# microsoft/protnote

Measured on AMD Instinct MI355X. Metric: protein-label pairs/sec (fwd+bwd), higher is better.
Workload: dtype f32

## Files before the change

### include/protnote_hip.h

```cpp
#ifndef PROTNOTE_HIP_H
#define PROTNOTE_HIP_H

#include <stddef.h>
#include <stdint.h>

#ifdef __cplusplus
extern "C" {
#endif

#define PN_MAX_BLOCKS 16
#define PN_MAX_LAYERS 8
#define PN_LABEL_F32 0
#define PN_LABEL_I64 1
#define PN_LABEL_U8 2

const char* pn_last_error(void);
int pn_version(void);
const char* pn_build_hash(void);

typedef struct pn_bn {
  const float* weight;
  const float* bias;
  float* running_mean;
  float* running_var;
// ... 179 lines not shown

#define PN_ADAM_WS_BYTES 32768
int pn_clip_adam_step(float* w, const float* g, float* m, float* v, long n, float max_norm, float lr, float beta1,
                      float beta2, float eps, float weight_decay, int step, float* norm_out, void* ws,
                      size_t ws_bytes, void* stream);

int pn_clip_sgd_step(float* w, const float* g, float* momentum_buf, long n, float max_norm, float lr, float momentum,
                     float weight_decay, int step, float* norm_out, void* ws, size_t ws_bytes, void* stream);

int pn_transpose(const float* src, long ld_src, int rows, int cols, float* dst, long ld_dst, void* stream);

int pn_gemm_tn(const float* A, long lda, const float* Bm, long ldb, float* C, long ldc, long R, int M, int N,
               void* ws, size_t ws_bytes, void* stream);

int pn_onehot_batch(const uint8_t* ids, const int64_t* offsets, int B, int A, int Lmax, float* onehots,
                    int64_t* lengths, void* stream);


int pn_ap_append(const float* scores, int ld_s, const void* labels, int label_kind, int ld_y, int B, int N_L,
                 uint32_t* keys, uint8_t* hits, long long cap, long long n0, void* stream);
size_t pn_ap_ws_bytes(int N_L, long long n, long long cap, int micro);
int pn_ap_compute(const uint32_t* keys, const uint8_t* hits, int N_L, long long n, long long cap, double* ap,
                  long long* npos, double* micro_ap, long long* micro_npos, void* ws, size_t ws_bytes, void* stream);

size_t pn_ap_partial_ws_bytes(long long m);
int pn_ap_partial(const uint32_t* keys, const uint8_t* hits, long long m, long long tp_before, long long k_before,
                  double* partial, long long* npos, void* ws, size_t ws_bytes, void* stream);

int pn_binned_hist_update(const float* scores, int ld_s, const void* labels, int label_kind, int ld_y, int B, int N_L,
                          const float* thresholds, int T, unsigned long long* pos_hist, unsigned long long* all_hist,
                          void* stream);
int pn_binned_auprc(unsigned long long* pos_hist, unsigned long long* all_hist, int N_L, int T, double* out,
                    long long* npos, int with_micro, void* stream);

int pn_set_math_mode(int mode);

int pn_set_mlp_materialize(int on);

typedef int (*pn_sync_hook)(long n_doubles, void* user);
int pn_set_sync_bn(pn_sync_hook hook, void* user, double* stage, long stage_doubles, int world);
int pn_get_math_mode(void);

int pn_set_backward_math(int mode);
int pn_get_backward_math(void);

int pn_set_forward_math(int mode);
int pn_get_forward_math(void);
int pn_set_fwd_staged(int on);
int pn_set_bf16_mfma16(int on);
int pn_set_bwd_deep(int mask);

int pn_set_f32_dma(int on);
int pn_set_b3_dma(int on);

int pn_set_encoder_f64(int on);

int pn_set_conv1_gather(int on);

int pn_dropout_mask(unsigned seed, int stream, float p, long rows, int cols, float* out, void* stream_);

int pn_prof_begin(void);
int pn_prof_end(int max_kinds, int* kinds, long* counts, double* total_ms, double* total_flops);

size_t pn_gemm_nt_stats_ws_bytes(int M, int N);
int pn_gemm_nt(const float* A, long lda, const float* W, long ldw, float* C, long ldc, int M, int N, int K,
               const float* bias, const float* a_scale, const float* a_shift, double* col_sum,
               double* col_sumsq, int tile_variant, void* ws, size_t ws_bytes, void* stream);

#ifdef __cplusplus
}
#endif
#endif
```

### protnote_amd/_lib.py

```python
import ctypes as C
import os

import torch

_HERE = os.path.dirname(os.path.abspath(__file__))
LIB_PATH = os.path.join(_HERE, "libprotnote_hip.so")

PN_MAX_BLOCKS = 16
PN_MAX_LAYERS = 8
PN_ADAM_WS_BYTES = 32768
fp = C.POINTER(C.c_float)


class pn_bn(C.Structure):
    _fields_ = [("weight", C.c_void_p), ("bias", C.c_void_p), ("running_mean", C.c_void_p),
                ("running_var", C.c_void_p)]


class pn_res_block(C.Structure):
    _fields_ = [("bn1", pn_bn), ("conv_a_w", C.c_void_p), ("conv_a_b", C.c_void_p), ("bn2", pn_bn),
                ("conv_b_w", C.c_void_p), ("conv_b_b", C.c_void_p)]


class pn_encoder(C.Structure):
# ... 108 lines not shown
    "pn_loss_fwd_bwd": (C.c_int, [C.c_void_p, C.c_void_p, C.c_void_p, C.c_int, C.c_int, C.c_int, C.c_float,
                                  C.c_float, C.c_float, C.c_float, C.c_float, C.c_void_p, C.c_void_p, C.c_void_p,
                                  C.c_void_p, C.c_void_p, C.c_int, C.c_void_p, C.c_float, C.c_void_p, C.c_size_t,
                                  C.c_void_p]),
    "pn_loss_fwd_bwd_t": (C.c_int, [C.c_void_p, C.c_void_p, C.c_int, C.c_int, C.c_int, C.c_int, C.c_float,
                                    C.c_float, C.c_float, C.c_float, C.c_float, C.c_void_p, C.c_void_p, C.c_void_p,
                                    C.c_void_p, C.c_void_p, C.c_int, C.c_void_p, C.c_float, C.c_void_p, C.c_size_t,
                                    C.c_void_p]),
    "pn_tp_fn_fp_t": (C.c_int, [C.c_void_p, C.c_void_p, C.c_int, C.c_int, C.c_int, C.c_float, C.c_void_p,
                                C.c_void_p, C.c_void_p, C.c_void_p]),
    "pn_supcon_ws_bytes": (C.c_size_t, [C.c_int]),
    "pn_supcon_fwd_bwd": (C.c_int, [C.c_void_p, C.c_void_p, C.c_void_p, C.c_int, C.c_int, C.c_void_p, C.c_void_p,
                                    C.c_void_p, C.c_size_t, C.c_void_p]),
    "pn_tp_fn_fp": (C.c_int, [C.c_void_p, C.c_void_p, C.c_void_p, C.c_int, C.c_int, C.c_float, C.c_void_p,
                              C.c_void_p, C.c_void_p, C.c_void_p]),
    "pn_clip_adam_step": (C.c_int, [C.c_void_p, C.c_void_p, C.c_void_p, C.c_void_p, C.c_long, C.c_float, C.c_float,
                                    C.c_float, C.c_float, C.c_float, C.c_float, C.c_int, C.c_void_p, C.c_void_p,
                                    C.c_size_t, C.c_void_p]),
    "pn_clip_sgd_step": (C.c_int, [C.c_void_p, C.c_void_p, C.c_void_p, C.c_long, C.c_float, C.c_float, C.c_float,
                                   C.c_float, C.c_int, C.c_void_p, C.c_void_p, C.c_size_t, C.c_void_p]),
    "pn_transpose": (C.c_int, [C.c_void_p, C.c_long, C.c_int, C.c_int, C.c_void_p, C.c_long, C.c_void_p]),
    "pn_gemm_tn": (C.c_int, [C.c_void_p, C.c_long, C.c_void_p, C.c_long, C.c_void_p, C.c_long, C.c_long, C.c_int,
                             C.c_int, C.c_void_p, C.c_size_t, C.c_void_p]),
    "pn_onehot_batch": (C.c_int, [C.c_void_p, C.c_void_p, C.c_int, C.c_int, C.c_int, C.c_void_p, C.c_void_p,
                                  C.c_void_p]),
    "pn_ap_append": (C.c_int, [C.c_void_p, C.c_int, C.c_void_p, C.c_int, C.c_int, C.c_int, C.c_int, C.c_void_p,
                               C.c_void_p, C.c_longlong, C.c_longlong, C.c_void_p]),
    "pn_ap_ws_bytes": (C.c_size_t, [C.c_int, C.c_longlong, C.c_longlong, C.c_int]),
    "pn_ap_compute": (C.c_int, [C.c_void_p, C.c_void_p, C.c_int, C.c_longlong, C.c_longlong, C.c_void_p, C.c_void_p,
                                C.c_void_p, C.c_void_p, C.c_void_p, C.c_size_t, C.c_void_p]),
    "pn_ap_partial_ws_bytes": (C.c_size_t, [C.c_longlong]),
    "pn_ap_partial": (C.c_int, [C.c_void_p, C.c_void_p, C.c_longlong, C.c_longlong, C.c_longlong, C.c_void_p, C.c_void_p,
                                C.c_void_p, C.c_size_t, C.c_void_p]),
    "pn_binned_hist_update": (C.c_int, [C.c_void_p, C.c_int, C.c_void_p, C.c_int, C.c_int, C.c_int, C.c_int,
                                        C.c_void_p, C.c_int, C.c_void_p, C.c_void_p, C.c_void_p]),
    "pn_binned_auprc": (C.c_int, [C.c_void_p, C.c_void_p, C.c_int, C.c_int, C.c_void_p, C.c_void_p, C.c_int,
                                  C.c_void_p]),
    "pn_dropout_mask": (C.c_int, [C.c_uint, C.c_int, C.c_float, C.c_long, C.c_int, C.c_void_p, C.c_void_p]),
    "pn_set_math_mode": (C.c_int, [C.c_int]),
    "pn_set_mlp_materialize": (C.c_int, [C.c_int]),
    "pn_set_sync_bn": (C.c_int, [C.c_void_p, C.c_void_p, C.c_void_p, C.c_long, C.c_int]),
    "pn_get_math_mode": (C.c_int, []),
    "pn_set_backward_math": (C.c_int, [C.c_int]),
    "pn_get_backward_math": (C.c_int, []),
    "pn_set_forward_math": (C.c_int, [C.c_int]),
    "pn_get_forward_math": (C.c_int, []),
    "pn_set_fwd_staged": (C.c_int, [C.c_int]),
    "pn_set_bf16_mfma16": (C.c_int, [C.c_int]),
    "pn_set_bwd_deep": (C.c_int, [C.c_int]),
    "pn_set_f32_dma": (C.c_int, [C.c_int]),
    "pn_set_encoder_f64": (C.c_int, [C.c_int]),
    "pn_set_conv1_gather": (C.c_int, [C.c_int]),
    "pn_set_b3_dma": (C.c_int, [C.c_int]),
    "pn_prof_begin": (C.c_int, []),
    "pn_prof_end": (C.c_int, [C.c_int, C.POINTER(C.c_int), C.POINTER(C.c_long), C.POINTER(C.c_double),
                              C.POINTER(C.c_double)]),
    "pn_gemm_nt": (C.c_int, [C.c_void_p, C.c_long, C.c_void_p, C.c_long, C.c_void_p, C.c_long, C.c_int, C.c_int,
                             C.c_int, C.c_void_p, C.c_void_p, C.c_void_p, C.c_void_p, C.c_void_p, C.c_int,
                             C.c_void_p, C.c_size_t, C.c_void_p]),
    "pn_gemm_nt_stats_ws_bytes": (C.c_size_t, [C.c_int, C.c_int]),
    "pn_loss_ws_bytes": (C.c_size_t, [C.c_int, C.c_int]),
}


def exported_symbols():
    return sorted(_SIGS)


def _ensure_current():
    from . import build

    have_src = os.path.isdir(build.CSRC) and os.path.exists(os.path.join(build.CSRC, "protnote_hip.hip"))
    if os.path.exists(LIB_PATH) and (not have_src or os.environ.get("PN_SKIP_HASH_CHECK") == "1"):
        return
    if os.path.exists(LIB_PATH) and not build.stale():
        return
    why = "is missing" if not os.path.exists(LIB_PATH) else (
        f"was built from other sources (binary {build.embedded_hash()}, csrc/ {build.csrc_hash()})")
    if not build.have_hipcc():
        raise RuntimeError(f"{LIB_PATH} {why} and hipcc is not available to rebuild it; build it with "
                           "`python -m protnote_amd.build` (protnote_amd has no CPU/eager fallback)")
    try:
        build.build_lib(verbose=False)
    except Exception as exc:
        raise RuntimeError(f"{LIB_PATH} {why} and could not be rebuilt ({exc}); build it with "
                           "`python -m protnote_amd.build` (protnote_amd has no CPU/eager fallback)") from exc


def build_hash() -> str:
    return lib().pn_build_hash().decode()


def lib():
    global _lib
    if _lib is None:
        _ensure_current()
        l = C.CDLL(LIB_PATH)
        for name, (res, args) in _SIGS.items():
            fn = getattr(l, name)
            fn.restype = res
            fn.argtypes = args
        _lib = l
        mode = os.environ.get("PN_MATH_MODE")
        if mode:
            set_math_mode(mode)
        mode = os.environ.get("PN_BACKWARD_MATH")
# ... 135 lines not shown
```

### protnote_amd/csrc/abi_heads_eval.hpp

```cpp
extern "C" size_t pn_mlp_rows_ws_bytes(const pn_mlp* m, int rows) {
  size_t b = 0;
  int hmax = 0;
  for (int i = 0; i + 1 < m->nlayers; ++i) hmax = m->dims[i + 1] > hmax ? m->dims[i + 1] : hmax;
  b += 2 * al256((size_t)rows * hmax * sizeof(float));
  b += 2 * al256((size_t)hmax * sizeof(float));
  return b;
}

extern "C" int pn_mlp_rows_fwd_eval(const pn_mlp* m, const float* x, int ldx, int rows, float* y, void* ws,
                                    size_t ws_bytes, void* stream) {
  PN_OK(math_field_check(m->math_mode, "pn_mlp_rows_fwd_eval"));
  MathScope math_scope(m->math_mode);
  hipStream_t st = (hipStream_t)stream;
  if (m->nlayers < 1 || m->nlayers > PN_MAX_LAYERS) return fail("mlp: bad layer count %d", m->nlayers);
  for (int i = 0; i <= m->nlayers; ++i)
    if (i < m->nlayers && m->dims[i] % 4 != 0) return fail("mlp: dims[%d]=%d not a multiple of 4", i, m->dims[i]);
  if (ldx % 4 != 0) return fail("mlp: ldx %% 4 != 0");
  int hmax = 0;
  for (int i = 0; i + 1 < m->nlayers; ++i) hmax = m->dims[i + 1] > hmax ? m->dims[i + 1] : hmax;
  Bump bp(ws, ws_bytes);
  float* buf[2];
  buf[0] = bp.take<float>((size_t)rows * hmax);
  buf[1] = bp.take<float>((size_t)rows * hmax);
  float* s = bp.take<float>(hmax);
// ... 452 lines not shown
    p.task_ns = ns;
    grid = dim3(tn_task_grid(ns), 1);
    if (SYNC && sync_ws != nullptr && ns * 4 * 4 <= TN_SYNC_INTS) {
      HIP_OK(hipMemsetAsync(sync_ws, 0, (size_t)ns * 4 * 4 * sizeof(int), st));
      p.task_sync = sync_ws;
    }
  }
  {
    ProfScope ps(100 + TA_PLAIN * 10 + TB, 2.0 * (double)R_all * (double)p.M * (double)p.N, st);
    hipLaunchKernelGGL(kern, grid, dim3(512), TN_FAST_LDS_BYTES, st, p);
    if (tail != 0) {
      auto tk = gemm_tn_kernel<TA_PLAIN, TB, false>;
      static bool tattr[64] = {false};
      if (dev < 64 && !tattr[dev]) {
        HIP_OK(hipFuncSetAttribute((const void*)tk, hipFuncAttributeMaxDynamicSharedMemorySize, TN_LDS_BYTES));
        tattr[dev] = true;
      }
      TnParams t = p;
      t.R = R_all; t.row_base = R_all - tail; t.rows_per_split = 32;
      t.Cpart = part + (size_t)ns * p.M * p.N; t.ldc = p.N; t.task_ns = 0; t.task_sync = nullptr;
      hipLaunchKernelGGL(tk, dim3((unsigned)((p.M / 128) * (p.N / 128)), 1), dim3(256), TN_LDS_BYTES, st, t);
    }
  }
  HIP_OK(hipGetLastError());
  if (ns > 1 || tail != 0) {
    hipLaunchKernelGGL(k_splitk_reduce, dim3(nblk((long)p.M * p.N, 256)), dim3(256), 0, st, (const float*)part,
                       ns + (tail != 0 ? 1 : 0), p.M, p.N, (long)p.N, dst, ldd);
    HIP_OK(hipGetLastError());
  }
  return 0;
}

template <int TB, int NP = 3, bool TR = false, bool ABF16 = false>
static int launch_tn_bf16x3(TnParams p, float* dst, long ldd, float* part, size_t part_cap_floats, hipStream_t st) {
  void (*kern)(TnParams) = nullptr;
  constexpr bool SYNC = TR && TB == TB_AFFINE_RELU;
  void (*kern_alt)(TnParams) = nullptr;
  if constexpr (TR) {
    kern = gemm_tn_bf16tr_kernel<TB, ABF16, SYNC, true>;
    kern_alt = gemm_tn_bf16tr_kernel<TB, ABF16, SYNC, false>;
  } else {
    kern = gemm_tn_bf16x3_kernel<TB, NP>;
  }
  constexpr int LDS = TR ? TN_BF16TR_LDS_BYTES : 2 * 512 * 36 * (int)sizeof(float);
  static std::atomic<bool> attr_done[64];
  int dev = 0;
  HIP_OK(hipGetDevice(&dev));
  if (dev < 64 && !attr_done[dev]) {
    HIP_OK(hipFuncSetAttribute((const void*)kern, hipFuncAttributeMaxDynamicSharedMemorySize, LDS));
    if (kern_alt != nullptr) HIP_OK(hipFuncSetAttribute((const void*)kern_alt, hipFuncAttributeMaxDynamicSharedMemorySize, LDS));
    attr_done[dev] = true;
  }
  if (kern_alt != nullptr && !g_bf16_m16.load()) kern = kern_alt;
  int ns = tn_pick_split(p.R, p.M, p.N, part_cap_floats, 256, 1);
  if (ns == 1) {
    p.Cpart = dst;
    p.ldc = ldd;
    p.rows_per_split = (p.R + 31) / 32 * 32;
  } else {
    if (part == nullptr) return fail("gemm_tn: no partial buffer");
    p.Cpart = part;
    p.ldc = p.N;
    long rps = (p.R + ns - 1) / ns;
    p.rows_per_split = (rps + 31) / 32 * 32;
    ns = (int)((p.R + p.rows_per_split - 1) / p.rows_per_split);
  }
  const unsigned tiles = (unsigned)((p.M / 256) * (p.N / 256));
  dim3 grid(tiles, (unsigned)ns);
  p.task_ns = 0;
  int* sync_ws = p.task_sync;
  p.task_sync = nullptr;
  if (p.M == 3072 && p.N == 3072 && ns >= 2) {
    p.task_ns = ns;
    grid = dim3(tn_task_grid(ns), 1);
    if (SYNC && sync_ws != nullptr && ns * 4 * 4 <= TN_SYNC_INTS) {
      HIP_OK(hipMemsetAsync(sync_ws, 0, (size_t)ns * 4 * 4 * sizeof(int), st));
      p.task_sync = sync_ws;
    }
  }
  {
    ProfScope ps((NP == 3 ? 1100 : 1600) + TB, 2.0 * (double)p.R * (double)p.M * (double)p.N, st);
    hipLaunchKernelGGL(kern, grid, dim3(512), LDS, st, p);
  }
  HIP_OK(hipGetLastError());
  if (ns > 1) {
    hipLaunchKernelGGL(k_splitk_reduce, dim3(nblk((long)p.M * p.N, 256)), dim3(256), 0, st, (const float*)part, ns,
                       p.M, p.N, (long)p.N, dst, ldd);
    HIP_OK(hipGetLastError());
  }
  return 0;
}

template <int TA, int TB>
static int launch_tn(TnParams p, float* dst, long ldd, float* part, size_t part_cap_floats, hipStream_t st) {
  if (p.M % 4 || p.N % 4) return fail("gemm_tn: M and N must be multiples of 4");
  if (p.R <= 0) return fail("gemm_tn: empty contraction");
  if (p.drop_thresh != 0) {
    if constexpr (TA == TA_PLAIN && (TB == TB_AFFINE_RELU || TB == TB_PAIRSUM_RELU)) {
      if (PN_BIG && use_f32_dma() && p.M % 256 == 0 && p.N % 256 == 0 && p.R >= 65536 && p.R % 32 == 0 && p.lda % 4 == 0)
        return launch_tn_cfg<TA, TB, true, true, true>(p, dst, ldd, part, part_cap_floats, st);
      return launch_tn_cfg<TA, TB, false, false, true>(p, dst, ldd, part, part_cap_floats, st);
    } else {
      return fail("gemm_tn: dropout is not defined for operand kinds %d x %d", TA, TB);
    }
  }
  if constexpr (TA == TA_PLAIN && (TB == TB_AFFINE_RELU || TB == TB_PAIRSUM_RELU)) {
// ... 59 lines not shown
```

### protnote_amd/csrc/protnote_hip.hip

```cpp
#include <hip/hip_runtime.h>
#include <stdarg.h>
#include <stdio.h>
#include <stdlib.h>
#include <string.h>

#include "../../include/protnote_hip.h"
#include "common.hpp"
#include "gemm_engine.hpp"
#include "gemm_bf16x3.hpp"
#include "gemm_bf16.hpp"
#include "gemm_dma.hpp"
#include "gemm_conv_dma.hpp"
#include "gemm_conv_f64.hpp"
#include "gemm_tn_fast.hpp"
#include "train_kernels.hpp"
#include "bwd_bf16_dz.hpp"
#include "fwd_bf16_h.hpp"
#include "gemm_bf16_m16.hpp"

using namespace pn;

static thread_local char g_err[512] = "";

static int fail(const char* fmt, ...) {
  va_list ap;
  va_start(ap, fmt);
  vsnprintf(g_err, sizeof(g_err), fmt, ap);
  va_end(ap);
  return 1;
}

#define HIP_OK(expr)                                                                         \
  do {                                                                                       \
    hipError_t _e = (expr);                                                                  \
    if (_e != hipSuccess) return fail("%s failed: %s (%s:%d)", #expr, hipGetErrorString(_e), \
                                      __FILE__, __LINE__);                                   \
  } while (0)
#define PN_OK(expr)         \
  do {                      \
    int _r = (expr);        \
    if (_r != 0) return _r; \
  } while (0)

int pn::fail_msg(const char* fmt, ...) {
  va_list ap;
  va_start(ap, fmt);
  vsnprintf(g_err, sizeof(g_err), fmt, ap);
  va_end(ap);
  return 1;
}

extern "C" const char* pn_last_error(void) { return g_err; }
extern "C" int pn_version(void) { return 1; }

static inline int ld4(int c) { return (c + 3) & ~3; }
static inline size_t al256(size_t b) { return (b + 255) & ~(size_t)255; }

struct Bump {
  char* base;
  size_t off, cap;
  bool ok;
  Bump(void* p, size_t cap_) : base((char*)p), off(0), cap(cap_), ok(true) {}
  template <class T>
  T* take(size_t n) {
    size_t b = al256(n * sizeof(T));
    if (off + b > cap) {
      ok = false;
      return nullptr;
    }
    T* r = (T*)(base + off);
    off += b;
// ... 255 lines not shown
  return 0;
}

static std::atomic<int> g_bwd_math{0};
extern "C" int pn_set_backward_math(int mode) {
  if (mode != 0 && mode != 1) return fail("pn_set_backward_math: 0 (as the forward) or 1 (bf16, one product)");
  g_bwd_math = mode;
  return 0;
}
extern "C" int pn_get_backward_math(void) { return g_bwd_math; }
static thread_local bool tl_bwd_bf16 = false;
static thread_local bool tl_dz_bf16 = false;
struct BwdBf16Scope {
  bool prev;
  explicit BwdBf16Scope(bool on) : prev(tl_bwd_bf16) { tl_bwd_bf16 = on; }
  ~BwdBf16Scope() {
    tl_bwd_bf16 = prev;
    tl_dz_bf16 = false;
  }
};

static std::atomic<int> g_fwd_math{0};
extern "C" int pn_set_forward_math(int mode) {
  if (mode != 0 && mode != 1) return fail("pn_set_forward_math: 0 (as math_mode) or 1 (bf16, one product)");
  g_fwd_math = mode;
  return 0;
}
extern "C" int pn_get_forward_math(void) { return g_fwd_math; }
static thread_local bool tl_fwd_bf16 = false;
struct FwdBf16Scope {
  bool prev;
  explicit FwdBf16Scope(bool on) : prev(tl_fwd_bf16) { tl_fwd_bf16 = on; }
  ~FwdBf16Scope() { tl_fwd_bf16 = prev; }
};
static bool fwd_bf16_requested(const pn_pairhead* hd) {
  const int m = hd->forward_math == 0 ? g_fwd_math.load(std::memory_order_relaxed) : hd->forward_math - 1;
  return m == 1 && hd->dropout_p == 0.f;
}
static int fwd_math_of(const pn_pairhead* hd, bool* bf16) {
  if (hd->forward_math < 0 || hd->forward_math > 2)
    return fail("pairhead: forward_math %d (0 = library default, 1 = as math_mode, 2 = bf16)", hd->forward_math);
  const int m = hd->forward_math == 0 ? g_fwd_math.load(std::memory_order_relaxed) : hd->forward_math - 1;
  *bf16 = (m == 1) && hd->dropout_p == 0.f;
  return 0;
}

static std::atomic<int> g_b3_dma{1};
static bool use_b3_dma() { return g_b3_dma == 1; }
extern "C" int pn_set_b3_dma(int on) {
  g_b3_dma = on ? 1 : 0;
  return 0;
}

template <int AK, int EK, int WAVES_N, int WN, bool GEN, bool BDMA = false, int NP = 3>
static int launch_gemm_bf16x3(const GemmParams& p, hipStream_t st) {
  using Cfg = GemmCfg<4, WAVES_N, 2, WN, 32>;
  if constexpr (!GEN && !BDMA && WAVES_N * WN * 32 == 256) {
    if (p.wsplit != nullptr && use_b3_dma() && p.Nstore == p.N)
      return launch_gemm_bf16x3<AK, EK, WAVES_N, WN, GEN, true>(p, st);
  }
  auto kern = gemm_nt_bf16x3_kernel<AK, EK, 4, WAVES_N, 2, WN, GEN, BDMA, NP>;
  constexpr int LDS_BYTES = BDMA ? 2 * (256 * 36 + 2 * 256 * 16) * (int)sizeof(float) : Cfg::LDS_BYTES;
  static std::atomic<bool> attr_done[64];
  int dev = 0;
  HIP_OK(hipGetDevice(&dev));
  if (dev < 64 && !attr_done[dev]) {
    HIP_OK(hipFuncSetAttribute((const void*)kern, hipFuncAttributeMaxDynamicSharedMemorySize, LDS_BYTES));
    attr_done[dev] = true;
  }
  if (p.M <= 0 || p.Nstore <= 0) return 0;
  if (p.Kseg % 4 != 0) return fail("gemm: K segment %d not a multiple of 4", p.Kseg);
  const long tm = (p.M + Cfg::BM - 1) / Cfg::BM;
  const long tn = (p.Nstore + Cfg::BN - 1) / Cfg::BN;
  GemmParams pp = p;
  pp.xcd_bc = (PN_XCD && tm >= 16) ? ((tn % 8 == 0) ? 8 : ((tn % 4 == 0) ? 4 : 0)) : 0;
  if (!GEN && AK == A_PAIRSUM_RELU && pp.xcd_bc && tm >= 64) pp.xcd_bc = 1;
  pp.xcd_br = pp.xcd_bc ? 32 / pp.xcd_bc : 0;
  long grid = tm * tn;
  if (pp.xcd_bc) {
    const long nblk = ((tm + pp.xcd_br - 1) / pp.xcd_br) * (tn / pp.xcd_bc);
    grid = ((nblk + 7) / 8) * 8 * 32;
  }
  if (grid > 0x7fffffffL) return fail("gemm: grid too large");
  if constexpr (BDMA) {
    pp.w_hi = p.wsplit;
    pp.w_lo = p.wsplit + (size_t)p.N * p.Kseg;
    hipLaunchKernelGGL(k_split_planes, dim3(nblk((long)p.N * p.Kseg / 4, 256)), dim3(256), 0, st, p.W, p.ldw, p.N, p.Kseg,
                       p.wsplit, p.wsplit + (size_t)p.N * p.Kseg);
  }
  {
    ProfScope ps((NP == 3 ? 1000 : 1500) + AK * 10 + EK, 2.0 * (double)p.M * (double)p.N * (double)p.nseg * (double)p.Kseg, st);
    hipLaunchKernelGGL(kern, dim3((unsigned)grid), dim3(Cfg::NT), LDS_BYTES, st, pp);
  }
  HIP_OK(hipGetLastError());
  return finish_col_stats(p, tm, st);
}

static std::atomic<int> g_bwd_deep{7};
extern "C" int pn_set_bwd_deep(int mask) {
  g_bwd_deep = mask & 7;
  return 0;
}
static int launch_gemm_bf16_single(const GemmParams& p, hipStream_t st) {
  auto kern = gemm_nt_bf16_kernel<E_STORE>;
  static std::atomic<bool> attr_done[64];
  int dev = 0;
  HIP_OK(hipGetDevice(&dev));
  if (dev < 64 && !attr_done[dev]) {
    HIP_OK(hipFuncSetAttribute((const void*)kern, hipFuncAttributeMaxDynamicSharedMemorySize, NT_BF16_LDS_BYTES));
    attr_done[dev] = true;
  }
  if (p.M <= 0 || p.Nstore <= 0) return 0;
  const long tm = (p.M + 255) / 256, tn = p.N / 256;
  GemmParams pp = p;
  pp.xcd_bc = (PN_XCD && tm >= 16) ? ((tn % 8 == 0) ? 8 : ((tn % 4 == 0) ? 4 : 0)) : 0;
  pp.xcd_br = pp.xcd_bc ? 32 / pp.xcd_bc : 0;
  long grid = tm * tn;
  if (pp.xcd_bc) {
    const long nblk_ = ((tm + pp.xcd_br - 1) / pp.xcd_br) * (tn / pp.xcd_bc);
    grid = ((nblk_ + 7) / 8) * 8 * 32;
  }
// ... 518 lines not shown
```

Measured before the change: 1.254 million.

## Add bf16x3 GEMM kernels using 16x16x32 MFMA with woven scheduling

Adds new NT and TN split-bf16 (bf16x3) GEMM kernels built on the 16x16x32 bf16 MFMA instruction. They use explicit sched_group_barrier weaving to interleave MFMA, VALU, LDS reads and writes, and double-buffer LDS with register prefetch. A global toggle, on by default, routes eligible shapes to these kernels. The aim is higher matrix-core throughput for the f32-emulating GEMMs, at the cost of extra code, register pressure and strict shape requirements (K multiple of 32, N multiple of 256).

```diff
diff --git a/include/protnote_hip.h b/include/protnote_hip.h
--- a/include/protnote_hip.h
+++ b/include/protnote_hip.h
@@ -255,6 +255,7 @@
 
 int pn_set_f32_dma(int on);
 int pn_set_b3_dma(int on);
+int pn_set_b3_mfma16(int on);
 
 int pn_set_encoder_f64(int on);
 
diff --git a/protnote_amd/_lib.py b/protnote_amd/_lib.py
--- a/protnote_amd/_lib.py
+++ b/protnote_amd/_lib.py
@@ -184,6 +184,7 @@
     "pn_set_encoder_f64": (C.c_int, [C.c_int]),
     "pn_set_conv1_gather": (C.c_int, [C.c_int]),
     "pn_set_b3_dma": (C.c_int, [C.c_int]),
+    "pn_set_b3_mfma16": (C.c_int, [C.c_int]),
     "pn_prof_begin": (C.c_int, []),
     "pn_prof_end": (C.c_int, [C.c_int, C.POINTER(C.c_int), C.POINTER(C.c_long), C.POINTER(C.c_double),
                               C.POINTER(C.c_double)]),
diff --git a/protnote_amd/csrc/abi_heads_eval.hpp b/protnote_amd/csrc/abi_heads_eval.hpp
--- a/protnote_amd/csrc/abi_heads_eval.hpp
+++ b/protnote_amd/csrc/abi_heads_eval.hpp
@@ -528,6 +528,14 @@
     attr_done[dev] = true;
   }
   if (kern_alt != nullptr && !g_bf16_m16.load()) kern = kern_alt;
+  if constexpr (!TR && NP == 3) {
+    static std::atomic<bool> attr16_done[64];
+    if (dev < 64 && !attr16_done[dev]) {
+      HIP_OK(hipFuncSetAttribute((const void*)gemm_tn_bf16x3_m16_kernel<TB>, hipFuncAttributeMaxDynamicSharedMemorySize, LDS));
+      attr16_done[dev] = true;
+    }
+    if (g_b3_m16.load()) kern = gemm_tn_bf16x3_m16_kernel<TB>;
+  }
   int ns = tn_pick_split(p.R, p.M, p.N, part_cap_floats, 256, 1);
   if (ns == 1) {
     p.Cpart = dst;
diff --git a/protnote_amd/csrc/gemm_bf16x3_m16.hpp b/protnote_amd/csrc/gemm_bf16x3_m16.hpp
--- /dev/null
+++ b/protnote_amd/csrc/gemm_bf16x3_m16.hpp
@@ -0,0 +1,560 @@
+#pragma once
+#include "gemm_bf16x3.hpp"
+#include "gemm_bf16_m16.hpp"
+
+#ifndef PN_B3M_VALU
+#define PN_B3M_VALU 2
+#endif
+
+namespace pn {
+
+template <int NV, int LEAD, bool RELOAD, bool WRITES>
+__device__ __forceinline__ void b3m_weave() {
+  if constexpr (LEAD > 0) __builtin_amdgcn_sched_group_barrier(0x100, LEAD, 0);
+#pragma unroll
+  for (int m = 0; m < 48; ++m) {
+    __builtin_amdgcn_sched_group_barrier(0x008, 1, 0);
+    if constexpr (NV > 0) __builtin_amdgcn_sched_group_barrier(0x002, NV, 0);
+    if (WRITES && m % 24 == 23) __builtin_amdgcn_sched_group_barrier(0x200, 2, 0);
+    if (RELOAD && m % 12 == 11) __builtin_amdgcn_sched_group_barrier(0x100, 2, 0);
+  }
+}
+
+#define PN_B3M_COL(ACC, J, AH, AL, BH, BL)                                                                      \
+  {                                                                                                             \
+    _Pragma("unroll") for (int i_ = 0; i_ < 4; ++i_)                                                            \
+        ACC[i_][J] = __builtin_amdgcn_mfma_f32_16x16x32_bf16(AL[i_], BH, ACC[i_][J], 0, 0, 0);                  \
+    _Pragma("unroll") for (int i_ = 0; i_ < 4; ++i_)                                                            \
+        ACC[i_][J] = __builtin_amdgcn_mfma_f32_16x16x32_bf16(AH[i_], BL, ACC[i_][J], 0, 0, 0);                  \
+    _Pragma("unroll") for (int i_ = 0; i_ < 4; ++i_)                                                            \
+        ACC[i_][J] = __builtin_amdgcn_mfma_f32_16x16x32_bf16(AH[i_], BH, ACC[i_][J], 0, 0, 0);                  \
+  }
+
+template <int AK, int EK, bool BDMA>
+__global__ __launch_bounds__(512, 2) void gemm_nt_bf16x3_m16_kernel(const GemmParams p) {
+  static_assert(AK == A_PLAIN || AK == A_AFFINE_RELU || AK == A_PAIRSUM_RELU, "operand kind not built for bf16x3");
+  static_assert(EK == E_STORE || EK == E_ROWDOT, "epilogue not covered by gemm_epilogue_m16");
+  constexpr int WAVES_M = 4, WAVES_N = 2, FM = 4, FN = 8;
+  constexpr int BK = 32, NT = 512, BM = 256, BN = 256;
+  constexpr int LDK = BK + 4;
+  constexpr int KV = BK / 8;
+  constexpr int RPP = NT / KV;
+  constexpr int NQ = BM / RPP;
+  constexpr int BPLANE = BN * 16;
+  constexpr int STAGE = BDMA ? BM * LDK + 2 * BPLANE : (BM + BN) * LDK;
+  constexpr int NV = AK == A_PLAIN ? PN_B3M_VALU : PN_B3M_VALU + 1;
+
+  extern __shared__ __attribute__((aligned(16))) float smem[];
+
+  const int tid = threadIdx.x;
+  const int lane = tid & 63;
+  const int wave = tid >> 6;
+  const int wm = wave / WAVES_N;
+  const int wn = wave % WAVES_N;
+
+  int tile_m, tile_n;
+  if (!tile_coords<BM, BN>(p, tile_m, tile_n)) return;
+  const int row0 = tile_m * BM;
+  const int col0 = tile_n * BN;
+
+  const uint16_t* bsrc[4] = {nullptr, nullptr, nullptr, nullptr};
+  unsigned bdst[4] = {0, 0, 0, 0};
+  if constexpr (BDMA) {
+    const int w = __builtin_amdgcn_readfirstlane(wave);
+#pragma unroll
+    for (int q = 0; q < 4; ++q) {
+      const int c = 4 * w + q;
+      const int r = 16 * (c & 15) + (lane >> 2);
+      const int g = (lane & 3) ^ ((r >> 2) & 3);
+      bsrc[q] = ((c >> 4) ? p.w_lo : p.w_hi) + (long)(col0 + r) * p.Kseg + 8 * g;
+      bdst[q] = (unsigned)(BM * LDK + (c >> 4) * BPLANE + 16 * (c & 15) * 16) * 4u;
+    }
+  }
+  const unsigned lds0_b = (unsigned)(uintptr_t)(const __attribute__((address_space(3))) float*)smem;
+  auto issue_b_dma = [&](int s_, int buf) {
+#pragma unroll
+    for (int q = 0; q < 4; ++q)
+      tn_glds16(reinterpret_cast<const float*>(bsrc[q] + s_ * BK),
+                __builtin_amdgcn_readfirstlane(lds0_b + (unsigned)(buf * STAGE) * 4u + bdst[q]));
+  };
+
+  const int kv = tid % KV;
+  const int r_in = tid / KV;
+
+  const float* arow[NQ];
+  const float* arow2[NQ];
+#pragma unroll
+  for (int q = 0; q < NQ; ++q) {
+    int r = row0 + r_in + q * RPP;
+    if (r > p.M - 1) r = p.M - 1;
+    if constexpr (AK == A_PAIRSUM_RELU) {
+      const int j = r / p.pairB;
+      const int i = r - j * p.pairB;
+      arow[q] = p.A + (long)i * p.lda + 4 * kv;
+      arow2[q] = p.A2 + (long)j * p.lda2 + 4 * kv;
+    } else {
+      arow[q] = p.A + (long)r * p.lda + 4 * kv;
+      arow2[q] = nullptr;
+    }
+  }
+  const float* brow[NQ];
+#pragma unroll
+  for (int q = 0; q < NQ; ++q) brow[q] = p.W + (long)(col0 + r_in + q * RPP) * p.ldw + 4 * kv;
+
+  const int nslab = p.Kseg / BK;
+
+  float4 ra[NQ][2], ra2[NQ][2], rb[NQ][2];
+  float4 rsc[2], rsh[2];
+
+  auto fetch_a = [&](int s) {
+    const int c = s * BK;
+#pragma unroll
+    for (int q = 0; q < NQ; ++q)
+#pragma unroll
+      for (int h = 0; h < 2; ++h) {
+        ra[q][h] = ld4(arow[q] + c + 16 * h);
+        if constexpr (AK == A_PAIRSUM_RELU) ra2[q][h] = ld4(arow2[q] + c + 16 * h);
+      }
+    if constexpr (AK == A_AFFINE_RELU) {
+#pragma unroll
+      for (int h = 0; h < 2; ++h) {
+        rsc[h] = ld4(p.a_scale + c + 4 * kv + 16 * h);
+        rsh[h] = ld4(p.a_shift + c + 4 * kv + 16 * h);
+      }
+    }
+  };
+  auto fetch_b = [&](int s) {
+    const int c = s * BK;
+#pragma unroll
+    for (int q = 0; q < NQ; ++q)
+#pragma unroll
+      for (int h = 0; h < 2; ++h) rb[q][h] = ld4(brow[q] + c + 16 * h);
+  };
+  auto pin_a = [&]() {
+#pragma unroll
+    for (int q = 0; q < NQ; ++q)
+#pragma unroll
+      for (int h = 0; h < 2; ++h) {
+        pin4(ra[q][h]);
+        if constexpr (AK == A_PAIRSUM_RELU) pin4(ra2[q][h]);
+      }
+  };
+  auto pin_b = [&]() {
+#pragma unroll
+    for (int q = 0; q < NQ; ++q)
+#pragma unroll
+      for (int h = 0; h < 2; ++h) pin4(rb[q][h]);
+  };
+
+  auto store8 = [](float* dst, float4 v0, float4 v1) {
+    const HiLo a = split4(v0), b = split4(v1);
+    bf16x8 hi, lo;
+#pragma unroll
+    for (int e = 0; e < 4; ++e) {
+      hi[e] = a.hi[e];
+      hi[4 + e] = b.hi[e];
+      lo[e] = a.lo[e];
+      lo[4 + e] = b.lo[e];
+    }
+    *reinterpret_cast<bf16x8*>(dst) = hi;
+    *reinterpret_cast<bf16x8*>(dst + 4) = lo;
+  };
+  auto commit_a = [&](int buf) {
+    float* As = smem + buf * STAGE;
+#pragma unroll
+    for (int q = 0; q < NQ; ++q) {
+      float4 v[2];
+#pragma unroll
+      for (int h = 0; h < 2; ++h) {
+        v[h] = ra[q][h];
+        if constexpr (AK == A_AFFINE_RELU) {
+          v[h].x = relu(fmaf(v[h].x, rsc[h].x, rsh[h].x));
+          v[h].y = relu(fmaf(v[h].y, rsc[h].y, rsh[h].y));
+          v[h].z = relu(fmaf(v[h].z, rsc[h].z, rsh[h].z));
+          v[h].w = relu(fmaf(v[h].w, rsc[h].w, rsh[h].w));
+        } else if constexpr (AK == A_PAIRSUM_RELU) {
+          v[h].x = relu(v[h].x + ra2[q][h].x);
+          v[h].y = relu(v[h].y + ra2[q][h].y);
+          v[h].z = relu(v[h].z + ra2[q][h].z);
+          v[h].w = relu(v[h].w + ra2[q][h].w);
+        }
+      }
+      store8(As + (r_in + q * RPP) * LDK + 8 * kv, v[0], v[1]);
+    }
+  };
+  auto commit_b = [&](int buf) {
+    float* Bs = smem + buf * STAGE + BM * LDK;
+#pragma unroll
+    for (int q = 0; q < NQ; ++q) store8(Bs + (r_in + q * RPP) * LDK + 8 * kv, rb[q][0], rb[q][1]);
+  };
+
+  f32x4 acc[FM][FN];
+#pragma unroll
+  for (int i = 0; i < FM; ++i)
+#pragma unroll
+    for (int j = 0; j < FN; ++j)
+#pragma unroll
+      for (int e = 0; e < 4; ++e) acc[i][j][e] = 0.f;
+
+  const int frow = lane & 15;
+  const int fg = lane >> 4;
+  const int a_off = (wm * FM * 16 + frow) * LDK + fg * 8;
+  constexpr int B_J = BDMA ? 16 * 16 : 16 * LDK;
+  constexpr int B_LO = BDMA ? BPLANE : 4;
+  const int b_off = BM * LDK + (BDMA ? (wn * FN * 16 + frow) * 16 + 4 * (fg ^ ((frow >> 2) & 3))
+                                     : (wn * FN * 16 + frow) * LDK + fg * 8);
+
+  bf16x8 ah[FM], al[FM], bh[4], bl[4];
+  auto region1 = [&](int buf) {
+    const float* As = smem + buf * STAGE + a_off;
+    const float* Bs = smem + buf * STAGE + b_off;
+#pragma unroll
+    for (int i = 0; i < FM; ++i) {
+      ah[i] = *reinterpret_cast<const bf16x8*>(As + i * 16 * LDK);
+      al[i] = *reinterpret_cast<const bf16x8*>(As + i * 16 * LDK + 4);
+    }
+#pragma unroll
+    for (int j = 0; j < 4; ++j) {
+      bh[j] = *reinterpret_cast<const bf16x8*>(Bs + j * B_J);
+      bl[j] = *reinterpret_cast<const bf16x8*>(Bs + j * B_J + B_LO);
+    }
+#pragma unroll
+    for (int j = 0; j < 4; ++j) {
+      PN_B3M_COL(acc, j, ah, al, bh[j], bl[j]);
+      bh[j] = *reinterpret_cast<const bf16x8*>(Bs + (j + 4) * B_J);
+      bl[j] = *reinterpret_cast<const bf16x8*>(Bs + (j + 4) * B_J + B_LO);
+    }
+  };
+  auto region2 = [&]() {
+#pragma unroll
+    for (int j = 0; j < 4; ++j) PN_B3M_COL(acc, j + 4, ah, al, bh[j], bl[j]);
+  };
+
+  if constexpr (BDMA) {
+    issue_b_dma(0, 0);
+    fetch_a(0);
+    pin_a();
+    commit_a(0);
+    fetch_a(nslab > 1 ? 1 : 0);
+    asm volatile("s_waitcnt vmcnt(0) lgkmcnt(0)" ::: "memory");
+    __builtin_amdgcn_s_barrier();
+    for (int s = 0; s + 1 < nslab; ++s) {
+      const int cur = s & 1;
+      const int nxt = s + 2 < nslab ? s + 2 : s + 1;
+      __builtin_amdgcn_sched_barrier(0);
+      pin_a();
+      issue_b_dma(s + 1, cur ^ 1);
+      __builtin_amdgcn_sched_barrier(0);
+      region1(cur);
+      commit_a(cur ^ 1);
+      b3m_weave<NV, 16, true, true>();
+      __builtin_amdgcn_sched_barrier(0);
+      asm volatile("s_waitcnt vmcnt(0)" ::: "memory");
+      fetch_a(nxt);
+      __builtin_amdgcn_sched_barrier(0);
+      region2();
+      __builtin_amdgcn_sched_barrier(0);
+      asm volatile("s_waitcnt lgkmcnt(0)" ::: "memory");
+      __builtin_amdgcn_s_barrier();
+    }
+    region1((nslab - 1) & 1);
+    __builtin_amdgcn_sched_barrier(0);
+    region2();
+    __syncthreads();
+  } else {
+    fetch_a(0);
+    fetch_b(0);
+    pin_a();
+    pin_b();
+    commit_a(0);
+    commit_b(0);
+    fetch_a(nslab > 1 ? 1 : 0);
+    fetch_b(nslab > 1 ? 1 : 0);
+    __syncthreads();
+    for (int s = 0; s + 1 < nslab; ++s) {
+      const int cur = s & 1;
+      const int nxt = s + 2 < nslab ? s + 2 : s + 1;
+      __builtin_amdgcn_sched_barrier(0);
+      pin_a();
+      region1(cur);
+      commit_a(cur ^ 1);
+      b3m_weave<NV, 16, true, true>();
+      __builtin_amdgcn_sched_barrier(0);
+      fetch_a(nxt);
+      __builtin_amdgcn_sched_barrier(0);
+      pin_b();
+      region2();
+      commit_b(cur ^ 1);
+      b3m_weave<PN_B3M_VALU, 0, false, true>();
+      __builtin_amdgcn_sched_barrier(0);
+      fetch_b(nxt);
+      __syncthreads();
+    }
+    region1((nslab - 1) & 1);
+    __builtin_amdgcn_sched_barrier(0);
+    region2();
+    __syncthreads();
+  }
+
+  gemm_epilogue_m16<EK, WAVES_M, WAVES_N, FM, FN>(p, acc, row0, col0, tile_n, smem);
+}
+
+template <int TB>
+__global__ __launch_bounds__(512, PN_MINW) void gemm_tn_bf16x3_m16_kernel(const TnParams p) {
+  constexpr int BM = 256, BN = 256, BK = 32, LDK = BK + 4;
+  constexpr int FM = 4, FN = 8;
+  constexpr int STAGE = (BM + BN) * LDK;
+  static_assert(TB == TB_PLAIN || TB == TB_AFFINE_RELU || TB == TB_PAIRSUM_RELU, "operand kind not built for bf16x3");
+
+  extern __shared__ __attribute__((aligned(16))) float smem[];
+
+  const int tid = threadIdx.x;
+  const int lane = tid & 63;
+  const int wave = tid >> 6;
+  const int wm = wave >> 1, wn = wave & 1;
+
+  const int ntn = p.N / BN, ntm = p.M / BM;
+  int tile_m, tile_n;
+  int split = blockIdx.y;
+  if (p.task_ns > 0) {
+    if (!tn_task_coords(p.task_ns, tile_m, tile_n, split)) return;
+  } else if (PN_XCD && TB == TB_PAIRSUM_RELU && (ntm % 4 == 0) && (ntn % 2 == 0)) {
+    const int rm = ntm / 4, rn = ntn / 2;
+    const int xcd = blockIdx.x & 7, w = blockIdx.x >> 3;
+    tile_m = (xcd >> 1) * rm + w / rn;
+    tile_n = (xcd & 1) * rn + w % rn;
+  } else if (PN_XCD && (ntm % 2 == 0) && (ntn % 4 == 0)) {
+    const int rm = ntm / 2, rn = ntn / 4;
+    const int xcd = blockIdx.x & 7, w = blockIdx.x >> 3;
+    tile_m = (xcd >> 2) * rm + w / rn;
+    tile_n = (xcd & 3) * rn + w % rn;
+  } else {
+    tile_n = blockIdx.x % ntn;
+    tile_m = blockIdx.x / ntn;
+  }
+  const int m0 = tile_m * BM, n0 = tile_n * BN;
+  const long r_begin = (long)split * p.rows_per_split;
+  long r_end = r_begin + p.rows_per_split;
+  if (r_end > p.R) r_end = p.R;
+
+  const int col = tid & 255;
+  const int kg = __builtin_amdgcn_readfirstlane(tid >> 8);
+  float bs = 0.f, bt = 0.f;
+  if constexpr (TB == TB_AFFINE_RELU) {
+    bs = p.b_s[n0 + col];
+    bt = p.b_t[n0 + col];
+  }
+
+  float ra[2][8], rb[2][8], rb2[2];
+  const unsigned pB = (unsigned)p.pairB;
+  const long lda = p.lda, ldb = p.ldb;
+
+  auto fetch_a = [&](long k0, auto safe_c) {
+    constexpr bool SAFE = decltype(safe_c)::value;
+    const float* Ak = p.A + k0 * lda + m0;
+    const int lim = (int)(r_end - 1 - k0);
+#pragma unroll
+    for (int g = 0; g < 2; ++g)
+#pragma unroll
+      for (int e = 0; e < 8; ++e) {
+        int ro = 8 * (kg + 2 * g) + e;
+        if (SAFE) ro = ro < lim ? ro : lim;
+        const float* rowp = Ak + (long)ro * lda;
+        ra[g][e] = rowp[(unsigned)col];
+      }
+  };
+  auto fetch_b = [&](long k0, auto safe_c) {
+    constexpr bool SAFE = decltype(safe_c)::value;
+    const int lim = (int)(r_end - 1 - k0);
+    if constexpr (TB == TB_PAIRSUM_RELU) {
+#pragma unroll
+      for (int g = 0; g < 2; ++g) {
+        int rr0 = 8 * (kg + 2 * g);
+        if (SAFE) rr0 = rr0 < lim ? rr0 : (lim & ~7);
+        const unsigned ru = (unsigned)(k0 + rr0);
+        const unsigned j = ru / pB;
+        const unsigned i = ru - j * pB;
+        const float* Bi = p.B + (long)i * ldb + n0;
+#pragma unroll
+        for (int e = 0; e < 8; ++e) {
+          int eo = e;
+          if (SAFE) eo = (rr0 + e) < lim ? e : (lim - rr0 > 0 ? lim - rr0 : 0);
+          const float* rowp = Bi + (long)eo * ldb;
+          rb[g][e] = rowp[(unsigned)col];
+        }
+        const float* B2j = p.B2 + (long)j * p.ldb2 + n0;
+        rb2[g] = B2j[(unsigned)col];
+      }
+    } else {
+      const float* Bk = p.B + k0 * ldb + n0;
+#pragma unroll
+      for (int g = 0; g < 2; ++g)
+#pragma unroll
+        for (int e = 0; e < 8; ++e) {
+          int ro = 8 * (kg + 2 * g) + e;
+          if (SAFE) ro = ro < lim ? ro : lim;
+          const float* rowp = Bk + (long)ro * ldb;
+          rb[g][e] = rowp[(unsigned)col];
+        }
+    }
+  };
+
+  auto pin_a = [&]() {
+#pragma unroll
+    for (int g = 0; g < 2; ++g)
+#pragma unroll
+      for (int e = 0; e < 8; ++e) asm volatile("" : "+v"(ra[g][e]));
+  };
+  auto pin_b = [&]() {
+#pragma unroll
+    for (int g = 0; g < 2; ++g) {
+#pragma unroll
+      for (int e = 0; e < 8; ++e) asm volatile("" : "+v"(rb[g][e]));
+      if constexpr (TB == TB_PAIRSUM_RELU) asm volatile("" : "+v"(rb2[g]));
+    }
+  };
+
+  auto store8 = [](float* dst, const float (&v)[8]) {
+    const HiLo a = split4(make_float4(v[0], v[1], v[2], v[3])), b = split4(make_float4(v[4], v[5], v[6], v[7]));
+    bf16x8 hi, lo;
+#pragma unroll
+    for (int e = 0; e < 4; ++e) {
+      hi[e] = a.hi[e];
+      hi[4 + e] = b.hi[e];
+      lo[e] = a.lo[e];
+      lo[4 + e] = b.lo[e];
+    }
+    *reinterpret_cast<bf16x8*>(dst) = hi;
+    *reinterpret_cast<bf16x8*>(dst + 4) = lo;
+  };
+
+  auto commit_a = [&](int buf, long k0, auto safe_c) {
+    constexpr bool SAFE = decltype(safe_c)::value;
+    float* As = smem + buf * STAGE;
+#pragma unroll
+    for (int g = 0; g < 2; ++g) {
+      float a[8];
+#pragma unroll
+      for (int e = 0; e < 8; ++e) {
+        a[e] = ra[g][e];
+        if (SAFE && k0 + 8 * (kg + 2 * g) + e >= r_end) a[e] = 0.f;
+      }
+      store8(As + col * LDK + 8 * (kg + 2 * g), a);
+    }
+  };
+  auto commit_b = [&](int buf, long k0, auto safe_c) {
+    constexpr bool SAFE = decltype(safe_c)::value;
+    float* Bs = smem + buf * STAGE + BM * LDK;
+#pragma unroll
+    for (int g = 0; g < 2; ++g) {
+      float b[8];
+#pragma unroll
+      for (int e = 0; e < 8; ++e) {
+        b[e] = rb[g][e];
+        if constexpr (TB == TB_AFFINE_RELU) b[e] = relu(fmaf(b[e], bs, bt));
+        if constexpr (TB == TB_PAIRSUM_RELU) b[e] = relu(b[e] + rb2[g]);
+        if (SAFE && k0 + 8 * (kg + 2 * g) + e >= r_end) b[e] = 0.f;
+      }
+      store8(Bs + col * LDK + 8 * (kg + 2 * g), b);
+    }
+  };
+
+  f32x4 acc[FM][FN];
+#pragma unroll
+  for (int i = 0; i < FM; ++i)
+#pragma unroll
+    for (int j = 0; j < FN; ++j)
+#pragma unroll
+      for (int e = 0; e < 4; ++e) acc[i][j][e] = 0.f;
+
+  const int frow = lane & 15;
+  const int fg = lane >> 4;
+  const int a_off = (wm * FM * 16 + frow) * LDK + fg * 8;
+  const int b_off = BM * LDK + (wn * FN * 16 + frow) * LDK + fg * 8;
+  bf16x8 ah[FM], al[FM], bh[4], bl[4];
+  auto region1 = [&](int buf) {
+    const float* As = smem + buf * STAGE + a_off;
+    const float* Bs = smem + buf * STAGE + b_off;
+#pragma unroll
+    for (int i = 0; i < FM; ++i) {
+      ah[i] = *reinterpret_cast<const bf16x8*>(As + i * 16 * LDK);
+      al[i] = *reinterpret_cast<const bf16x8*>(As + i * 16 * LDK + 4);
+    }
+#pragma unroll
+    for (int j = 0; j < 4; ++j) {
+      bh[j] = *reinterpret_cast<const bf16x8*>(Bs + j * 16 * LDK);
+      bl[j] = *reinterpret_cast<const bf16x8*>(Bs + j * 16 * LDK + 4);
+    }
+#pragma unroll
+    for (int j = 0; j < 4; ++j) {
+      PN_B3M_COL(acc, j, ah, al, bh[j], bl[j]);
+      bh[j] = *reinterpret_cast<const bf16x8*>(Bs + (j + 4) * 16 * LDK);
+      bl[j] = *reinterpret_cast<const bf16x8*>(Bs + (j + 4) * 16 * LDK + 4);
+    }
+  };
+  auto region2 = [&]() {
+#pragma unroll
+    for (int j = 0; j < 4; ++j) PN_B3M_COL(acc, j + 4, ah, al, bh[j], bl[j]);
+  };
+
+  using std::false_type;
+  using std::true_type;
+  if (r_begin < r_end) {
+    const long span = r_end - r_begin;
+    const int nf = (int)(span / BK);
+    const int ns = nf + ((span % BK) ? 1 : 0);
+    auto K0 = [&](int t) { return r_begin + (long)t * BK; };
+    auto body = [&](int t, auto safe_c) {
+      const int cur = t & 1;
+      const int t2 = t + 2 < ns ? t + 2 : t + 1;
+      __builtin_amdgcn_sched_barrier(0);
+      pin_a();
+      region1(cur);
+      commit_a(cur ^ 1, K0(t + 1), safe_c);
+      b3m_weave<1, 16, true, true>();
+      __builtin_amdgcn_sched_barrier(0);
+      fetch_a(K0(t2), safe_c);
+      __builtin_amdgcn_sched_barrier(0);
+      pin_b();
+      region2();
+      commit_b(cur ^ 1, K0(t + 1), safe_c);
+      b3m_weave<(TB == TB_PLAIN ? 1 : 2), 0, false, true>();
+      __builtin_amdgcn_sched_barrier(0);
+      fetch_b(K0(t2), safe_c);
+      __syncthreads();
+    };
+    fetch_a(K0(0), true_type{});
+    fetch_b(K0(0), true_type{});
+    pin_a();
+    pin_b();
+    commit_a(0, K0(0), true_type{});
+    commit_b(0, K0(0), true_type{});
+    fetch_a(K0(ns > 1 ? 1 : 0), true_type{});
+    fetch_b(K0(ns > 1 ? 1 : 0), true_type{});
+    __syncthreads();
+    int t = 0;
+    for (; t + 2 < nf; ++t) body(t, false_type{});
+    for (; t + 1 < ns; ++t) body(t, true_type{});
+    region1((ns - 1) & 1);
+    __builtin_amdgcn_sched_barrier(0);
+    region2();
+  }
+
+  float* out = p.Cpart + (long)split * p.M * p.ldc;
+  const int rq = lane >> 4;
+#pragma unroll
+  for (int i = 0; i < FM; ++i)
+#pragma unroll
+    for (int j = 0; j < FN; ++j) {
+      const int n = n0 + (wn * FN + j) * 16 + frow;
+#pragma unroll
+      for (int e = 0; e < 4; ++e) {
+        const int m = m0 + (wm * FM + i) * 16 + 4 * rq + e;
+        out[(long)m * p.ldc + n] = acc[i][j][e];
+      }
+    }
+}
+
+#undef PN_B3M_COL
+
+}
diff --git a/protnote_amd/csrc/protnote_hip.hip b/protnote_amd/csrc/protnote_hip.hip
--- a/protnote_amd/csrc/protnote_hip.hip
+++ b/protnote_amd/csrc/protnote_hip.hip
@@ -17,6 +17,7 @@
 #include "bwd_bf16_dz.hpp"
 #include "fwd_bf16_h.hpp"
 #include "gemm_bf16_m16.hpp"
+#include "gemm_bf16x3_m16.hpp"
 
 using namespace pn;
 
@@ -378,6 +379,12 @@
   return 0;
 }
 
+static std::atomic<int> g_b3_m16{1};
+extern "C" int pn_set_b3_mfma16(int on) {
+  g_b3_m16 = on ? 1 : 0;
+  return 0;
+}
+
 template <int AK, int EK, int WAVES_N, int WN, bool GEN, bool BDMA = false, int NP = 3>
 static int launch_gemm_bf16x3(const GemmParams& p, hipStream_t st) {
   using Cfg = GemmCfg<4, WAVES_N, 2, WN, 32>;
@@ -385,14 +392,20 @@
     if (p.wsplit != nullptr && use_b3_dma() && p.Nstore == p.N)
       return launch_gemm_bf16x3<AK, EK, WAVES_N, WN, GEN, true>(p, st);
   }
-  auto kern = gemm_nt_bf16x3_kernel<AK, EK, 4, WAVES_N, 2, WN, GEN, BDMA, NP>;
+  void (*kern)(GemmParams) = gemm_nt_bf16x3_kernel<AK, EK, 4, WAVES_N, 2, WN, GEN, BDMA, NP>;
   constexpr int LDS_BYTES = BDMA ? 2 * (256 * 36 + 2 * 256 * 16) * (int)sizeof(float) : Cfg::LDS_BYTES;
+  constexpr bool HAS_M16 = !GEN && NP == 3 && WAVES_N * WN * 32 == 256 && (EK == E_STORE || EK == E_ROWDOT);
   static std::atomic<bool> attr_done[64];
   int dev = 0;
   HIP_OK(hipGetDevice(&dev));
   if (dev < 64 && !attr_done[dev]) {
     HIP_OK(hipFuncSetAttribute((const void*)kern, hipFuncAttributeMaxDynamicSharedMemorySize, LDS_BYTES));
+    if constexpr (HAS_M16)
+      HIP_OK(hipFuncSetAttribute((const void*)gemm_nt_bf16x3_m16_kernel<AK, EK, BDMA>, hipFuncAttributeMaxDynamicSharedMemorySize, LDS_BYTES));
     attr_done[dev] = true;
+  }
+  if constexpr (HAS_M16) {
+    if (g_b3_m16.load() && p.Kseg % 32 == 0 && p.N % 256 == 0 && p.nseg == 1) kern = gemm_nt_bf16x3_m16_kernel<AK, EK, BDMA>;
   }
   if (p.M <= 0 || p.Nstore <= 0) return 0;
   if (p.Kseg % 4 != 0) return fail("gemm: K segment %d not a multiple of 4", p.Kseg);
```

New measurement: 1.255 million (median of 3 runs). No clear change (+0.1%).
